# peterhpark/neuroclear

Measured on AMD Instinct MI355X. Metric: voxels/sec, higher is better.
Workload: dtype f32

## Files before the change

### include/nc_hip.h

```cpp
#ifndef NC_HIP_H
#define NC_HIP_H

#include <stddef.h>
#include <stdint.h>

#ifdef __cplusplus
extern "C" {
#endif

#define NC_OK 0
#define NC_ERR_SHAPE (-1)
#define NC_ERR_WS (-2)
#define NC_ERR_HIP (-3)
#define NC_ERR_ARG (-4)

const char* nc_last_error(void);
int nc_version(void);
int nc_conv_fwd_path(int C, int K, int kd, int kh, int kw, int stride, int pad);
int nc_conv_wgrad_path(int C, int K, int kd, int kh, int kw, int stride, int pad);
void nc_prof_begin(double min_flop);
int nc_prof_end(int max, int* cls, double* flop, float* ms);
int nc_prof_end2(int max, int* cls, double* flop, float* ms, double* abytes);
void nc_set_force_direct(int on);
void nc_sconv_set_cfg(int cfg);
// ... 146 lines not shown
size_t nc_unet_deconv_param_floats(void);
size_t nc_unet_deconv_saved_floats(int N, int S0, int S1, int S2);
size_t nc_unet_deconv_train_ws_bytes(int N, int S0, int S1, int S2);
int nc_unet_deconv_train_fwd(const float* params, const float* x, float* y, float* saved, int N, int S0, int S1, int S2,
                             void* ws, size_t ws_bytes, void* stream, unsigned* kept);
int nc_unet_deconv_bwd(const float* params, const float* x, const float* y, const float* saved, const float* dy, float* dx,
                       float* dparams, int N, int S0, int S1, int S2, void* ws, size_t ws_bytes, void* stream, unsigned kept);
void nc_set_unet_lean(int on);
int nc_get_unet_lean(void);
void nc_set_unet_wprep(int on);
int nc_get_unet_wprep(void);
int nc_unet_wprep_layout(int N, int S0, int S1, int S2, int block, int form, size_t* pack_off, size_t* pack_bytes, size_t* cell_off,
                         size_t* bound_off);
int nc_s3x_pack_h2_debug(const float* w, int C, int K, int form, const unsigned* cell_a, const unsigned* cell_b, void* wp, unsigned* wcell,
                         void* stream);
int nc_convT_h2_bound_debug(const float* w, const float* bias, int C, int K, float in_bound, unsigned* cell, void* stream);
size_t nc_deep_linear_param_floats(void);
size_t nc_deep_linear_saved_floats(int N, int S0, int S1, int S2);
size_t nc_deep_linear_ws_bytes(int N, int S0, int S1, int S2);
int nc_deep_linear_fwd(const float* params, const float* x, float* y, float* saved , int N, int S0, int S1,
                       int S2, void* ws, size_t ws_bytes, void* stream, unsigned* kept );
void nc_set_dl_collapse(int on);
int nc_get_dl_collapse(void);
int nc_deep_linear_bwd(const float* params, const float* x, const float* saved, const float* dy, float* dx, float* dparams,
                       int N, int S0, int S1, int S2, void* ws, size_t ws_bytes, void* stream, unsigned kept);

int nc_conv_fwd_c8(const void* xh, const float* w, const float* bias, void* yh, int out_ctot, int out_c0, int N, int C, int D, int H,
                   int W, int K, int kd, int kh, int kw, int stride, int pad, int dtype, void* ws, size_t ws_bytes, void* stream);
int nc_conv_dgrad_c8(const void* dyh, const float* w, void* dxh, int N, int C, int D, int H, int W, int K, int kd, int kh, int kw,
                     int stride, int pad, int dtype, void* ws, size_t ws_bytes, void* stream);
size_t nc_conv_c1_c8_ws_bytes(int N, int D, int H, int W, int ks);
int nc_conv_c1_fwd_c8(const float* x, const float* w, const float* bias, void* yh, int out_ctot, int out_c0, int N, int D, int H, int W,
                      int ks, int dtype, void* ws, size_t ws_bytes, void* stream);
int nc_conv_c1_dgrad_c8(const void* dyh, const float* w, float* dx, int N, int D, int H, int W, int ks, void* ws, size_t ws_bytes,
                        void* stream);
size_t nc_conv_c1_wgrad_c8_ws_bytes(int N, int D, int H, int W, int ks);
int nc_conv_c1_wgrad_c8(const float* x, const void* dyh, float* dw, int N, int D, int H, int W, int ks, void* ws, size_t ws_bytes,
                        void* stream);
size_t nc_c8_instnorm_ws_bytes(int N, int C, long S);
int nc_c8_instnorm_stats(const void* xh, int N, int C, long S, float eps, float* mean, float* rstd, int dtype, void* ws,
                         size_t ws_bytes, void* stream);
int nc_c8_instnorm_act_fwd(const void* xh, const float* mean, const float* rstd, float slope, void* yh, int out_ctot, int out_c0,
                           int N, int C, long S, int dtype, void* stream);
int nc_c8_instnorm_act_bwd(const void* gh, int g_ctot, int g_c0, const void* xh, const float* mean, const float* rstd, float slope,
                           void* dxh, float* dbias , int N, int C, long S, int dtype, void* ws, size_t ws_bytes,
                           void* stream);
// ... 99 lines not shown
```

### neuroclear_amd/_lib.py

```python
import ctypes
import os
import re

_HERE = os.path.dirname(os.path.abspath(__file__))
LIB_PATH = os.environ.get('NC_HIP_LIB') or os.path.join(_HERE, 'csrc', 'libnc_hip.so')
HEADER_PATH = os.path.join(os.path.dirname(_HERE), 'include', 'nc_hip.h')

_lib = None


class NcError(RuntimeError):
    pass


def header_symbols():
    src = open(HEADER_PATH).read()
    src = re.sub(r'/\*.*?\*/', '', src, flags=re.S)
    return sorted(set(re.findall(r'\b(nc_[a-zA-Z0-9_]+)\s*\(', src)))


def lib():
    global _lib
    if _lib is None:
        if not os.path.exists(LIB_PATH):
            raise NcError('libnc_hip.so is not built (%s): run `python -c "import __graft_entry__ as g; g.build()"` '
                          'or `make -C neuroclear_amd/csrc`; there is no CPU fallback' % LIB_PATH)
        L = ctypes.CDLL(LIB_PATH)
        for name in header_symbols():
            fn = getattr(L, name)
            if name.endswith('_bytes') or name.endswith('_floats') or name == 'nc_h2_cells_offset':
                fn.restype = ctypes.c_size_t
            elif name == 'nc_last_error':
                fn.restype = ctypes.c_char_p
            elif name in ('nc_set_force_direct', 'nc_prof_begin', 'nc_sconv_set_cfg', 'nc_sconv_set_tune', 'nc_set_conv_split', 'nc_set_s3_fusion', 'nc_set_c8x_mode', 'nc_set_split_terms', 'nc_set_h2_guard', 'nc_set_epi_stats', 'nc_set_dl_collapse', 'nc_set_p2d_terms', 'nc_set_s3x_w64', 'nc_set_unet_lean', 'nc_set_unet_wprep'):
                fn.restype = None
            else:
                fn.restype = ctypes.c_int
        _lib = L
    return _lib


def check(code, what=''):
    if code != 0:
        raise NcError('%s failed (%d): %s' % (what, code, lib().nc_last_error().decode()))


P = ctypes.c_void_p
I = ctypes.c_int
L_ = ctypes.c_long
F = ctypes.c_float
Z = ctypes.c_size_t
```

### neuroclear_amd/csrc/common.hpp

```cpp
#pragma once
#include <hip/hip_runtime.h>

#include <cstdarg>
#include <cstdio>

#include "../../include/nc_hip.h"

namespace nc {

void set_error(const char* fmt, ...);

inline int check_launch(const char* what) {
  hipError_t e = hipGetLastError();
  if (e != hipSuccess) {
    set_error("%s: %s", what, hipGetErrorString(e));
    return NC_ERR_HIP;
  }
  return NC_OK;
}

inline long cdiv(long a, long b) { return (a + b - 1) / b; }

int raise_dyn_lds(const void* kernel, int bytes, const char* who);
template <typename K>
// ... 174 lines not shown
struct WPrepSeg { const float* w; int Cin, Kout, flip; unsigned a_bits; int b_cell; unsigned* ext_cell; };
struct WPrepBound { const float* w; const float* bias; int C, K; float in_bound; int cell; };
size_t wprep_bytes(const WPrepSeg* segs, int n);
int wprep_run(const WPrepSeg* segs, int n, const WPrepBound* bounds, int nb, void* region, S3xPrepared* out, hipStream_t s);
int s3x_pack_h2(const float* w, int Cin, int Kout, int KS, long so, long si, int flip, int split_c, const unsigned* cell_a, const unsigned* cell_b,
                unsigned* wcell, void* wp_ws, hipStream_t s);
void s3x_set_terms(int t);
int s3x_get_terms();
int conv_s3x_h2(const void* xs, const unsigned* cell_a, const unsigned* cell_b, int split_c, const float* w, const float* bias, float* y, int N,
                int Cin, int D, int H, int W, int Kout, int KS, long so, long si, int flip, unsigned* wcell, void* wp_ws, hipStream_t s,
                const unsigned* guard = nullptr, float* stats_part = nullptr, const S3xPrepared* prep = nullptr);
size_t s3x_stats_bytes(int N, int D, int H, int W, int Kout, int KS);
int s3x_stats_finalize(const float* stats_part, const float* bias, int N, int D, int H, int W, int Kout, int KS, float eps, float* mean, float* rstd,
                       hipStream_t s);
bool c1k7_h2_supported(const ConvDims& d);
size_t c1k7_h2_ws_bytes(const ConvDims& d);
int conv_c1k7_h2(const float* x, const float* w, const float* bias, float* y, const ConvDims& d, void* ws, size_t wsb, hipStream_t s);
size_t c1k7_h2_dgrad_ws_bytes(const ConvDims& d);
bool dl_typed_supported(int N, int D, int H, int W);
size_t dl_typed_bytes(int N, int D, int H, int W);
const float* dl_typed_wp(const char* scratch, int N, int D, int H, int W);
float* dl_typed_dwsw(char* scratch, int N, int D, int H, int W);
int dl_typed_compose(const float* F, char* scratch, int N, int D, int H, int W, hipStream_t s);
int dl_typed_fwd_boundary(const float* act0, float* y, char* scratch, int N, int D, int H, int W, hipStream_t s);
int dl_typed_dgrad_boundary(const float* act0, const float* dy, float* g, char* scratch, int N, int D, int H, int W, hipStream_t s);
int dl_typed_p(const float* act0, const float* dy, float* Pq, char* scratch, int N, int D, int H, int W, hipStream_t s);
int conv_c1k7_h2_dgrad(const float* dy, const float* w, float* dx, const ConvDims& d, void* ws, size_t wsb, hipStream_t s);
inline size_t h2_cells_offset(size_t elems) { return (elems * 4 + 255) & ~(size_t)255; }
inline unsigned* h2_cells_of(const void* t, size_t elems) { return (unsigned*)((char*)const_cast<void*>(t) + h2_cells_offset(elems)); }
int instnorm_relu_tail_sigmoid(const float* x, const float* mean, const float* rstd, const float* w1, const float* b1, const float* w2,
                               const float* b2, float* y, int C, long S, hipStream_t s);
int instnorm_act_bwd_dbias_h2(const float* dy, const float* x, const float* mean, const float* rstd, float slope, void* dxs,
                              float* dbias, int N, int C, long S, void* ws, size_t ws_bytes, void* stream, unsigned* guard = nullptr);
int instnorm_act_bwd_dbias_h2_rank1(const float* dy1, const float* w1, const float* x, const float* mean, const float* rstd, float slope, void* dxs,
                                    float* dbias, int C, long S, void* ws, size_t ws_bytes, void* stream, unsigned* guard);
unsigned* conv_bwd_guard_words(void* ws, int N, int K, long S);
int maxpool2_h2(const void* in, void* out, int N, int C, int ctot, int D, int H, int W, hipStream_t s);
int h2_zero_cells(unsigned* cells, int n, hipStream_t s);
int h2_set_cell(unsigned* cell, float bound, hipStream_t s);
int h2_absmax(const float* x, long n, unsigned* cell, hipStream_t s, unsigned* cell2 = nullptr);
int split2h_into(const float* x, long xstride, void* xs, int N, int C, long S, int ctot, int c0, const unsigned* cell, hipStream_t s,
                 unsigned* guard = nullptr);
constexpr int kGuardLow = 0, kGuardAll = 1, kGuardFlag = 2;
constexpr unsigned kGuardDrop = 17u << 23;
constexpr unsigned long long kGuardShare = 64;
#if defined(__HIP_DEVICE_COMPILE__)
__device__ __forceinline__ bool guard_skip(const unsigned* guard, int want) {
  return guard && (int)(__builtin_nontemporal_load(guard + kGuardFlag) != 0) != want;
}
// ... 113 lines not shown
```

### neuroclear_amd/csrc/dl_typed.hip

```cpp
#include "common.hpp"

namespace nc {
namespace {

constexpr int kT = 27, kD7 = 343, kC = 64;

__host__ __device__ inline int axis_type(int coord, int L) { return coord == 0 ? 0 : coord == L - 1 ? 2 : 1; }
__host__ __device__ inline bool tap_ok(int ta, int t) { return !((ta == 0 && t == 0) || (ta == 2 && t == 2)); }

__global__ void __launch_bounds__(64) k_dl_h_from_f(const float* __restrict__ F, float* __restrict__ Hc, float* __restrict__ Hd, float* __restrict__ Wp,
                                                    float* __restrict__ Hr, float* __restrict__ Hx) {
  const int tau = blockIdx.x, d = blockIdx.y, c = threadIdx.x;
  const int dz = d / 49, dy = (d / 7) % 7, dx = d % 7;
  const int tz_ = tau / 9, ty_ = (tau / 3) % 3, tx_ = tau % 3;
  double v = 0.0, v13 = 0.0;
  for (int tz = 0; tz < 3; ++tz) {
    const int sz = dz - tz;
    if (sz < 0 || sz > 4) continue;
    for (int ty = 0; ty < 3; ++ty) {
      const int sy = dy - ty;
      if (sy < 0 || sy > 4) continue;
      for (int tx = 0; tx < 3; ++tx) {
        const int sx = dx - tx;
        if (sx < 0 || sx > 4) continue;
// ... 347 lines not shown
  const int tau = blockIdx.y;
  const long i = (long)blockIdx.x * 256 + threadIdx.x;
  if (i >= (long)kD7 * kC) return;
  const int tz = tau / 9, ty = (tau / 3) % 3, tx = tau % 3;
  double v = 0.0;
  if (tau != 13) {
    for (int n = 0; n < N; ++n) {
      if (tx == 1) {
        int r0, cnt, st;
        if (tz != 1) { const int b = tz == 0 ? 0 : H; r0 = b + (ty == 0 ? 0 : ty == 2 ? H - 1 : 1); cnt = ty == 1 ? H - 2 : 1; st = 1; }
        else { r0 = 2 * H + (ty == 2 ? 1 : 0); cnt = D - 2; st = 2; }
        for (int j = 0; j < cnt; ++j) v += (double)partA[((long)n * nrows + r0 + (long)j * st) * kD7 * kC + i];
      } else {
        const int side = tx >> 1;
        const long slot = (long)N * 2 * D * kD7 * kC;
        const int z0 = tz == 0 ? 0 : tz == 2 ? D - 1 : 1, cnt = tz == 1 ? D - 2 : 1;
        for (int j = 0; j < cnt; ++j) v += (double)partB[(long)ty * slot + (((long)n * 2 + side) * D + z0 + j) * kD7 * kC + i];
      }
    }
  }
  dHb[(long)tau * kD7 * kC + i] = (float)v;
}

size_t al256(size_t b) { return (b + 255) & ~(size_t)255; }

}

struct DlTyped {
  size_t Hc, Hd, Wp, dWsw, dHb, AX, dyX, partA, partB, Hr, Hx, total;
  int nrows;
};
static DlTyped dl_typed_plan(int N, int D, int H, int W) {
  DlTyped t{};
  size_t off = 0;
  auto take = [&](size_t b) { const size_t r = off; off += al256(b); return r; };
  t.nrows = n_bnd_rows(D, H);
  t.Hc = take((size_t)kT * kD7 * kC * 4); t.Hd = take((size_t)kT * kD7 * kC * 4); t.Wp = take((size_t)kC * kD7 * 4); t.dWsw = take((size_t)kC * kD7 * 4);
  t.dHb = take((size_t)kT * kD7 * kC * 4);
  t.AX = take((size_t)N * 2 * kC * D * 4 * H * 4); t.dyX = take((size_t)N * 2 * D * H * 4);
  t.Hr = take((size_t)kT * 49 * kC * 8 * 4); t.Hx = take((size_t)kT * 49 * kC * 8 * 4);
  t.partA = take((size_t)N * t.nrows * kD7 * kC * 4); t.partB = take((size_t)3 * N * 2 * D * kD7 * kC * 4);
  t.total = off;
  return t;
}
bool dl_typed_supported(int N, int D, int H, int W) {
  return N >= 1 && D >= 8 && H >= 8 && W >= 8 && H <= 192 && W <= 192 && W % 4 == 0;
}
size_t dl_typed_bytes(int N, int D, int H, int W) { return dl_typed_supported(N, D, H, W) ? dl_typed_plan(N, D, H, W).total : 0; }
const float* dl_typed_wp(const char* scratch, int N, int D, int H, int W) { return (const float*)(scratch + dl_typed_plan(N, D, H, W).Wp); }
float* dl_typed_dwsw(char* scratch, int N, int D, int H, int W) { return (float*)(scratch + dl_typed_plan(N, D, H, W).dWsw); }

int dl_typed_compose(const float* F, char* scratch, int N, int D, int H, int W, hipStream_t s) {
  const DlTyped t = dl_typed_plan(N, D, H, W);
  hipLaunchKernelGGL(k_dl_h_from_f, dim3(kT, kD7), dim3(64), 0, s, F, (float*)(scratch + t.Hc), (float*)(scratch + t.Hd), (float*)(scratch + t.Wp), (float*)(scratch + t.Hr),
                     (float*)(scratch + t.Hx));
  return check_launch("deep_linear: typed kernels");
}
int dl_typed_fwd_boundary(const float* act0, float* y, char* scratch, int N, int D, int H, int W, hipStream_t s) {
  const DlTyped t = dl_typed_plan(N, D, H, W);
  float* AX = (float*)(scratch + t.AX);
  hipLaunchKernelGGL(k_dl_gather_x, dim3((unsigned)D, kC, (unsigned)(N * 2)), dim3(128), 0, s, act0, AX, (const float*)nullptr, (float*)nullptr, D, H, W);
  hipLaunchKernelGGL(k_dl_bnd_fwd<false>, dim3((unsigned)t.nrows, (unsigned)cdiv(W - 2, kSeg), (unsigned)N), dim3(448), 0, s, act0, (const float*)(scratch + t.Hr), y, D, H, W);
  hipLaunchKernelGGL(k_dl_bnd_fwd<true>, dim3((unsigned)D, (unsigned)(2 * cdiv(H - 2, kSeg)), (unsigned)N), dim3(448), 0, s, (const float*)AX, (const float*)(scratch + t.Hx), y,
                     D, H, W);
  hipLaunchKernelGGL(k_dl_bnd_fwd_ends, dim3((unsigned)D, 4, (unsigned)N), dim3(256), 0, s, (const float*)AX, (const float*)(scratch + t.Hc), y, D, H, W);
  return check_launch("deep_linear: typed forward, boundary");
}
int dl_typed_dgrad_boundary(const float* act0, const float* dy, float* g, char* scratch, int N, int D, int H, int W, hipStream_t s) {
  const DlTyped t = dl_typed_plan(N, D, H, W);
  float* AX = (float*)(scratch + t.AX);
  float* dyX = (float*)(scratch + t.dyX);
  hipLaunchKernelGGL(k_dl_gather_x, dim3((unsigned)D, kC, (unsigned)(N * 2)), dim3(128), 0, s, act0, AX, dy, dyX, D, H, W);
  hipLaunchKernelGGL(k_dl_bnd_dgrad<false>, dim3((unsigned)(D * H), (unsigned)cdiv(W, 64), (unsigned)N), dim3(256), 0, s, dy, (const float*)(scratch + t.Hd), g, D, H, W, 1);
  const int nseg = (int)cdiv(H, 64);
  hipLaunchKernelGGL(k_dl_bnd_dgrad<true>, dim3((unsigned)D, 2, (unsigned)(N * nseg)), dim3(256), 0, s, (const float*)dyX, (const float*)(scratch + t.Hd), g, D, H, W, nseg);
  hipLaunchKernelGGL(k_dl_bnd_dgrad_ends, dim3((unsigned)D, 4, (unsigned)N), dim3(256), 0, s, (const float*)dyX, (const float*)(scratch + t.Hd), g, D, H, W);
  return check_launch("deep_linear: typed data gradient, boundary");
}
int dl_typed_p(const float* act0, const float* dy, float* Pq, char* scratch, int N, int D, int H, int W, hipStream_t s) {
  const DlTyped t = dl_typed_plan(N, D, H, W);
  const float* AX = (const float*)(scratch + t.AX);
  const float* dyX = (const float*)(scratch + t.dyX);
  const size_t lds = (size_t)(64 * kPitch + 192) * 4;
  hipLaunchKernelGGL(k_dl_bnd_wgrad<false>, dim3((unsigned)t.nrows, 7, (unsigned)N), dim3(448), lds, s, act0, dy, (float*)(scratch + t.partA), D, H, W, t.nrows);
  hipLaunchKernelGGL(k_dl_bnd_wgrad<true>, dim3((unsigned)(2 * D), 7, (unsigned)N), dim3(448), lds, s, AX, dyX, (float*)(scratch + t.partB), D, H, W, t.nrows);
  hipLaunchKernelGGL(k_dl_bnd_reduce, dim3((unsigned)cdiv((long)kD7 * kC, 256), kT), dim3(256), 0, s, (const float*)(scratch + t.partA), (const float*)(scratch + t.partB),
                     (float*)(scratch + t.dHb), N, D, H, W, t.nrows);
  hipLaunchKernelGGL(k_dl_p_from_dh, dim3(kC, 32), dim3(128), 0, s, (const float*)(scratch + t.dWsw), (const float*)(scratch + t.dHb), Pq);
  return check_launch("deep_linear: typed parameter gradients");
}

}
```

### neuroclear_amd/csrc/gen_nets.hip

```cpp

#include <atomic>
#include <cstdlib>

#include "common.hpp"

using namespace nc;

#define NC_TRY(expr) do { int e_ = (expr); if (e_) return e_; } while (0)

namespace {

size_t up64(size_t n) { return (n + 63) & ~(size_t)63; }

size_t s3_floats(size_t elems) { return up64((elems * 6 + 3) / 4); }
size_t align256(size_t b) { return (b + 255) & ~(size_t)255; }

std::atomic<int> g_unet_lean{getenv("NC_UNET_LEAN") ? (atoi(getenv("NC_UNET_LEAN")) != 0) : 1};
constexpr int kLeanBit0 = 10;
constexpr int kLeanBlocks[5] = {1, 3, 5, 6, 8};
int lean_index(int consumer) {
  for (int j = 0; j < 5; ++j) if (kLeanBlocks[j] == consumer) return j;
  return -1;
}

// ... 586 lines not shown
  const int t = threadIdx.x;
  const double* a = (const double*)(tail + LTail::a);
  const double* r = (const double*)(tail + LTail::r);
  for (int i = t; i < 32 * 64; i += 256) dw3[i] = (float)(a[i / 64] * r[i % 64]);
  if (t < 32) {
    double v = 0.0;
    for (int c = 0; c < 64; ++c) v += (double)w3[t * 64 + c] * r[c];
    ss[t] = v;
  }
  __syncthreads();
  for (int i = t; i < 16 * 32; i += 256) dw4[i] = (float)((double)w5[i / 32] * ss[i % 32]);
  if (t < 16) {
    double v = 0.0;
    for (int b = 0; b < 32; ++b) v += (double)w4[t * 32 + b] * ss[b];
    dw5[t] = (float)v;
  }
}

std::atomic<int> g_dl_collapse{getenv("NC_DL_COLLAPSE") ? (atoi(getenv("NC_DL_COLLAPSE")) < 0 ? 0 : atoi(getenv("NC_DL_COLLAPSE")) > 2 ? 2 : atoi(getenv("NC_DL_COLLAPSE"))) : 2};

}

namespace nc {
bool dl_collapse_on() { return g_dl_collapse.load(std::memory_order_relaxed) != 0; }
size_t dl_tail_bytes() { return LTail::bytes; }
const float* dl_tail_E(const char* tail) { return (const float*)(tail + LTail::E); }
const float* dl_tail_Ef(const char* tail) { return (const float*)(tail + LTail::Ef); }
float* dl_tail_q(char* tail) { return (float*)(tail + LTail::q); }
int dl_tail_compose(const float* w2, const float* w3, const float* w4, const float* w5, char* tail, hipStream_t s) {
  hipLaunchKernelGGL(k_dl_compose, dim3(8), dim3(256), 0, s, w2, w3, w4, w5, tail);
  return check_launch("deep_linear: compose");
}
float* dl_tail_P(char* tail) { return (float*)(tail + LTail::P); }
const float* dl_w1_fold(char* tail, const float* w1, hipStream_t s) {
  hipLaunchKernelGGL(k_dl_w1_fold, dim3(64, 32), dim3(128), 0, s, (const float*)(tail + LTail::E), w1, (float*)(tail + LTail::Wf));
  return check_launch("deep_linear_bwd: composed data-gradient weights") ? nullptr : (const float*)(tail + LTail::Wf);
}
const float* dl_fold_fwd64(char* tail, const float* w1, hipStream_t s) {
  static_assert(LTail::Wf == LTail::P + (size_t)64 * 32 * 125 * 4 + 256, "P and Wf adjacent");
  float* F = (float*)(tail + LTail::P);
  if (hipMemsetAsync(F + (size_t)32 * 64 * 125, 0, (size_t)32 * 64 * 125 * 4, s) != hipSuccess) return nullptr;
  hipLaunchKernelGGL(k_dl_fold_fwd, dim3(32, 64), dim3(128), 0, s, (const float*)(tail + LTail::E), w1, F);
  return check_launch("deep_linear_fwd: composed forward weights") ? nullptr : F;
}
int dl_combine27(const float* Z, float* y, int N, int D, int H, int W, int zch, hipStream_t s) {
  hipLaunchKernelGGL(k_dl_combine27, dim3(1024, (unsigned)N), dim3(256), 0, s, Z, y, D, H, W, zch);
// ... 44 lines not shown
  return true;
}

}

extern "C" {

size_t nc_deep_linear_param_floats(void) {
  LPlan p;
  l_plan(p, 1, 8, 8, 8);
  return p.params;
}

size_t nc_deep_linear_saved_floats(int N, int S0, int S1, int S2) {
  LPlan p;
  return l_plan(p, N, S0, S1, S2) ? p.saved : 0;
}

size_t nc_deep_linear_ws_bytes(int N, int S0, int S1, int S2) {
  LPlan p;
  return l_plan(p, N, S0, S1, S2) ? align256(p.conv_ws) + p.grads * sizeof(float) + 256 + align256(LTail::bytes) + dl_typed_bytes(N, S0, S1, S2) : 0;
}

void nc_set_dl_collapse(int on) { g_dl_collapse.store(on < 0 ? 0 : on > 2 ? 2 : on, std::memory_order_relaxed); }
int nc_get_dl_collapse(void) { return g_dl_collapse.load(std::memory_order_relaxed); }

int nc_deep_linear_fwd(const float* params, const float* x, float* y, float* saved, int N, int S0, int S1, int S2, void* ws,
                       size_t ws_bytes, void* stream, unsigned* kept) {
  NetworkScope net_scope;
  if (!params || !x || !y) { set_error("deep_linear_fwd: null pointer"); return NC_ERR_ARG; }
  LPlan p;
  if (!l_plan(p, N, S0, S1, S2)) { set_error("deep_linear_fwd: bad shape"); return NC_ERR_SHAPE; }
  if (!ws || ws_bytes < nc_deep_linear_ws_bytes(N, S0, S1, S2)) { set_error("deep_linear_fwd: workspace too small"); return NC_ERR_WS; }
  void* cws = ws;
  float* G = (float*)((char*)ws + align256(p.conv_ws));
  const float* in = x;
  unsigned kept_mask = 0;
  if (kept) *kept = 0;
  const bool collapse = g_dl_collapse.load(std::memory_order_relaxed) != 0;
  char* tail = (char*)ws + align256(p.conv_ws) + p.grads * sizeof(float) + 256;
  hipStream_t hs = (hipStream_t)stream;
  static const bool k32_on = !(getenv("NC_DL_K32") && atoi(getenv("NC_DL_K32")) == 0);
  char* typed = tail + align256(LTail::bytes);
  ConvDims d0;
  const bool typed_ok = g_dl_collapse.load(std::memory_order_relaxed) == 2 && saved && dl_typed_supported(N, S0, S1, S2) && make_dims(d0, N, 1, S0, S1, S2, 64, 7, 7, 7, 1, 3) && c1k7_h2_supported(d0) &&
                        c1_wgrad_supported(d0) && c1k7_h2_dgrad_ws_bytes(d0) <= p.conv_ws && c1k7_h2_ws_bytes(d0) <= p.conv_ws &&
                        c1_wgrad_ws_bytes(d0) <= p.conv_ws;
  for (int i = 0; i < 6; ++i) {
    ConvDims dk;
    if (typed_ok && i == 1) {
      hipLaunchKernelGGL(k_dl_compose, dim3(8), dim3(256), 0, hs, params + p.w[2], params + p.w[3], params + p.w[4], params + p.w[5], tail);
      hipLaunchKernelGGL(k_dl_fold_fwd, dim3(32, 64), dim3(128), 0, hs, (const float*)(tail + LTail::E), params + p.w[1], (float*)(tail + LTail::Wf));
      NC_TRY(check_launch("deep_linear_fwd: composed kernels"));
      NC_TRY(dl_typed_compose((const float*)(tail + LTail::Wf), typed, N, S0, S1, S2, hs));
      NC_TRY(conv_c1k7_h2_dgrad(in, dl_typed_wp(typed, N, S0, S1, S2), y, d0, cws, p.conv_ws, hs));
      NC_TRY(dl_typed_fwd_boundary(in, y, typed, N, S0, S1, S2, hs));
      kept_mask |= kKeptCollapsed | kKeptNoAct1 | kKeptTyped;
      break;
    }
    if (collapse && i == 1 && saved && k32_on && make_dims(dk, N, 64, S0, S1, S2, 32, 5, 5, 5, 1, 2) && conv_fwd_h2_k32_supported(dk) &&
        (size_t)256 + s3x_packed_bytes(64, 32, 5, 2) + 512 <= p.conv_ws) {
      hipLaunchKernelGGL(k_dl_compose, dim3(8), dim3(256), 0, hs, params + p.w[2], params + p.w[3], params + p.w[4], params + p.w[5], tail);
      hipLaunchKernelGGL(k_dl_fold_fwd, dim3(32, 64), dim3(128), 0, hs, (const float*)(tail + LTail::E), params + p.w[1], (float*)(tail + LTail::Wf));
      NC_TRY(check_launch("deep_linear_fwd: composed forward weights"));
      float* Z = saved + p.act[1];
      NC_TRY(conv_fwd_h2_k32_keep(in, (const float*)(tail + LTail::Wf), Z, dk, cws, p.conv_ws, hs, saved + p.xs3[1]));
      hipLaunchKernelGGL(k_dl_combine27, dim3(1024, (unsigned)N), dim3(256), 0, hs, (const float*)Z, y, S0, S1, S2, 32);
      NC_TRY(check_launch("deep_linear_fwd: shifted sum"));
      kept_mask |= kKeptCollapsed | kKeptNoAct1 | (1u << 1) | (1u << 17);
      break;
    }
    if (collapse && i == 2) {
      hipLaunchKernelGGL(k_dl_compose, dim3(8), dim3(256), 0, hs, params + p.w[2], params + p.w[3], params + p.w[4], params + p.w[5], tail);
      NC_TRY(check_launch("deep_linear_fwd: compose"));
      NC_TRY(conv_fwd_to1_k3(in, (const float*)(tail + LTail::E), y, N, 64, S0, S1, S2, cws, p.conv_ws, hs));
      kept_mask |= kKeptCollapsed;
      break;
    }
    const LLayer& l = kLL[i];
// ... 18 lines not shown
  NetworkScope net_scope;
  if (!params || !x || !saved || !dy || !dparams) { set_error("deep_linear_bwd: null pointer"); return NC_ERR_ARG; }
  LPlan p;
  if (!l_plan(p, N, S0, S1, S2)) { set_error("deep_linear_bwd: bad shape"); return NC_ERR_SHAPE; }
  if (!ws || ws_bytes < nc_deep_linear_ws_bytes(N, S0, S1, S2)) { set_error("deep_linear_bwd: workspace too small"); return NC_ERR_WS; }
  void* cws = ws;
  float* G = (float*)((char*)ws + align256(p.conv_ws));
  const float* g = dy;
  const unsigned kept_mask = kept;
  int top = 5;
  ConvDims dsh, cd1;
  static const bool rank_on = !(getenv("NC_DL_RANK_WGRAD") && atoi(getenv("NC_DL_RANK_WGRAD")) == 0);
  static const bool rank_dg_on = !(getenv("NC_DL_RANK_DGRAD") && atoi(getenv("NC_DL_RANK_DGRAD")) == 0);
  const bool h2_1 = make_dims(cd1, N, 64, S0, S1, S2, 64, 5, 5, 5, 1, 2) && conv_layer_h2(cd1);
  const bool have1 = ((kept_mask >> 1) & 1) && ((kept_mask >> 17) & 1) != 0;
  const bool rank_w = (kept_mask & kKeptCollapsed) && rank_on && h2_1 && have1 && make_dims(dsh, N, 32, S0, S1, S2, 64, 5, 5, 5, 1, 2) &&
                      wgrad_h2_supported(dsh) && s3_wgrad_ws_bytes(dsh) <= p.conv_ws;
  const bool rank_dgrad = rank_w && rank_dg_on && conv_fwd_h2_c32_supported(dsh) && conv_fwd_h2_c32_ws_bytes(dsh) <= p.conv_ws;
  const bool rank_all = rank_dgrad;
  if (kept_mask & kKeptTyped) {
    hipStream_t hs = (hipStream_t)stream;
    char* tail = (char*)ws + align256(p.conv_ws) + p.grads * sizeof(float) + 256;
    char* typed = tail + align256(LTail::bytes);
    ConvDims d0;
    ForceTwoTerm two_;
    if (!dl_typed_supported(N, S0, S1, S2) || !make_dims(d0, N, 1, S0, S1, S2, 64, 7, 7, 7, 1, 3) || !c1k7_h2_supported(d0) || !c1_wgrad_supported(d0)) {
      set_error("deep_linear_bwd: the forward ran the position-typed form, which this shape does not admit");
      return NC_ERR_ARG;
    }
    const float* act0 = saved + p.act[0];
    hipLaunchKernelGGL(k_dl_compose, dim3(8), dim3(256), 0, hs, params + p.w[2], params + p.w[3], params + p.w[4], params + p.w[5], tail);
    hipLaunchKernelGGL(k_dl_fold_fwd, dim3(32, 64), dim3(128), 0, hs, (const float*)(tail + LTail::E), params + p.w[1], (float*)(tail + LTail::Wf));
    NC_TRY(check_launch("deep_linear_bwd: composed kernels"));
    NC_TRY(dl_typed_compose((const float*)(tail + LTail::Wf), typed, N, S0, S1, S2, hs));
    float* g0 = G + p.g[1];
    NC_TRY(conv_c1k7_h2(dy, dl_typed_wp(typed, N, S0, S1, S2), nullptr, g0, d0, cws, p.conv_ws, hs));
    NC_TRY(dl_typed_dgrad_boundary(act0, dy, g0, typed, N, S0, S1, S2, hs));
    NC_TRY(conv_wgrad_c1(dy, act0, dl_typed_dwsw(typed, N, S0, S1, S2), d0, cws, p.conv_ws, hs));
    NC_TRY(dl_typed_p(act0, dy, (float*)(tail + LTail::P), typed, N, S0, S1, S2, hs));
    hipLaunchKernelGGL(k_dl_q_from_p, dim3(64, 27), dim3(256), 0, hs, params + p.w[1], (const float*)(tail + LTail::P), (float*)(tail + LTail::q));
    hipLaunchKernelGGL(k_dl_w1_contract, dim3(64, 64), dim3(128), 0, hs, (const float*)(tail + LTail::E), (const float*)(tail + LTail::P), dparams + p.w[1]);
    hipLaunchKernelGGL(k_dl_tail_w2, dim3(64), dim3(256), 0, hs, params + p.w[2], tail, dparams + p.w[2]);
    hipLaunchKernelGGL(k_dl_tail_w345, dim3(1), dim3(256), 0, hs, params + p.w[3], params + p.w[4], params + p.w[5], (const char*)tail, dparams + p.w[3],
                       dparams + p.w[4], dparams + p.w[5]);
    NC_TRY(check_launch("deep_linear_bwd: typed parameter gradients"));
    g = g0;
    top = 0;
  } else if (kept_mask & kKeptCollapsed) {
    hipStream_t hs = (hipStream_t)stream;
    char* tail = (char*)ws + align256(p.conv_ws) + p.grads * sizeof(float) + 256;
    const float* act1 = saved + p.act[1];
    hipLaunchKernelGGL(k_dl_compose, dim3(8), dim3(256), 0, hs, params + p.w[2], params + p.w[3], params + p.w[4], params + p.w[5], tail);
    NC_TRY(check_launch("deep_linear_bwd: compose"));
    if (rank_w) {
      float* Dsh = G + p.g[1];
      hipLaunchKernelGGL(k_dl_shift27, dim3(256, 32, (unsigned)N), dim3(256), 0, hs, dy, Dsh, S0, S1, S2);
      NC_TRY(check_launch("deep_linear_bwd: shifted copies of dy"));
      NC_TRY(conv_wgrad_h2(Dsh, nullptr, nullptr, saved + p.xs3[1], (float*)(tail + LTail::P), dsh, cws, p.conv_ws, hs));
      hipLaunchKernelGGL(k_dl_q_from_p, dim3(64, 27), dim3(256), 0, hs, params + p.w[1], (const float*)(tail + LTail::P), (float*)(tail + LTail::q));
      hipLaunchKernelGGL(k_dl_w1_contract, dim3(64, 64), dim3(128), 0, hs, (const float*)(tail + LTail::E), (const float*)(tail + LTail::P), dparams + p.w[1]);
      NC_TRY(check_launch("deep_linear_bwd: q, dW1"));
    } else {
// ... 50 lines not shown
```

Baseline: 55.04 million.

## Group boundary rows in typed deep-linear boundary kernels to reuse line loads

Adds grouped variants of the boundary forward, data-gradient and weight-gradient kernels for the position-typed deep-linear path. Each block now handles several adjacent boundary rows (kG=4) and reuses the loaded input lines and window shifts across them, instead of one row per block. The grouped path is on by default behind a new toggle. In exchange it uses more registers and LDS per block, adds decode logic, and runs fewer blocks.

```diff
diff --git a/include/nc_hip.h b/include/nc_hip.h
--- a/include/nc_hip.h
+++ b/include/nc_hip.h
@@ -192,6 +192,8 @@
                        int S2, void* ws, size_t ws_bytes, void* stream, unsigned* kept );
 void nc_set_dl_collapse(int on);
 int nc_get_dl_collapse(void);
+void nc_set_dl_bnd(int on);
+int nc_get_dl_bnd(void);
 int nc_deep_linear_bwd(const float* params, const float* x, const float* saved, const float* dy, float* dx, float* dparams,
                        int N, int S0, int S1, int S2, void* ws, size_t ws_bytes, void* stream, unsigned kept);
 
diff --git a/neuroclear_amd/_lib.py b/neuroclear_amd/_lib.py
--- a/neuroclear_amd/_lib.py
+++ b/neuroclear_amd/_lib.py
@@ -32,7 +32,7 @@
                 fn.restype = ctypes.c_size_t
             elif name == 'nc_last_error':
                 fn.restype = ctypes.c_char_p
-            elif name in ('nc_set_force_direct', 'nc_prof_begin', 'nc_sconv_set_cfg', 'nc_sconv_set_tune', 'nc_set_conv_split', 'nc_set_s3_fusion', 'nc_set_c8x_mode', 'nc_set_split_terms', 'nc_set_h2_guard', 'nc_set_epi_stats', 'nc_set_dl_collapse', 'nc_set_p2d_terms', 'nc_set_s3x_w64', 'nc_set_unet_lean', 'nc_set_unet_wprep'):
+            elif name in ('nc_set_force_direct', 'nc_prof_begin', 'nc_sconv_set_cfg', 'nc_sconv_set_tune', 'nc_set_conv_split', 'nc_set_s3_fusion', 'nc_set_c8x_mode', 'nc_set_split_terms', 'nc_set_h2_guard', 'nc_set_epi_stats', 'nc_set_dl_collapse', 'nc_set_p2d_terms', 'nc_set_s3x_w64', 'nc_set_unet_lean', 'nc_set_unet_wprep', 'nc_set_dl_bnd'):
                 fn.restype = None
             else:
                 fn.restype = ctypes.c_int
diff --git a/neuroclear_amd/csrc/common.hpp b/neuroclear_amd/csrc/common.hpp
--- a/neuroclear_amd/csrc/common.hpp
+++ b/neuroclear_amd/csrc/common.hpp
@@ -220,9 +220,9 @@
 const float* dl_typed_wp(const char* scratch, int N, int D, int H, int W);
 float* dl_typed_dwsw(char* scratch, int N, int D, int H, int W);
 int dl_typed_compose(const float* F, char* scratch, int N, int D, int H, int W, hipStream_t s);
-int dl_typed_fwd_boundary(const float* act0, float* y, char* scratch, int N, int D, int H, int W, hipStream_t s);
-int dl_typed_dgrad_boundary(const float* act0, const float* dy, float* g, char* scratch, int N, int D, int H, int W, hipStream_t s);
-int dl_typed_p(const float* act0, const float* dy, float* Pq, char* scratch, int N, int D, int H, int W, hipStream_t s);
+int dl_typed_fwd_boundary(const float* act0, float* y, char* scratch, int N, int D, int H, int W, bool groups, hipStream_t s);
+int dl_typed_dgrad_boundary(const float* act0, const float* dy, float* g, char* scratch, int N, int D, int H, int W, bool groups, hipStream_t s);
+int dl_typed_p(const float* act0, const float* dy, float* Pq, char* scratch, int N, int D, int H, int W, bool groups, hipStream_t s);
 int conv_c1k7_h2_dgrad(const float* dy, const float* w, float* dx, const ConvDims& d, void* ws, size_t wsb, hipStream_t s);
 inline size_t h2_cells_offset(size_t elems) { return (elems * 4 + 255) & ~(size_t)255; }
 inline unsigned* h2_cells_of(const void* t, size_t elems) { return (unsigned*)((char*)const_cast<void*>(t) + h2_cells_offset(elems)); }
diff --git a/neuroclear_amd/csrc/dl_typed.hip b/neuroclear_amd/csrc/dl_typed.hip
--- a/neuroclear_amd/csrc/dl_typed.hip
+++ b/neuroclear_amd/csrc/dl_typed.hip
@@ -393,6 +393,335 @@
   dHb[(long)tau * kD7 * kC + i] = (float)v;
 }
 
+constexpr int kG = 4;
+__device__ __forceinline__ int wave_id() { return __builtin_amdgcn_readfirstlane((int)(threadIdx.x >> 6)); }
+__host__ __device__ inline int n_groups(int L) { return (L - 2 + kG - 1) / kG; }
+__host__ __device__ inline int n_ygroups(int H) { return 2 * n_groups(H) + 4; }
+__host__ __device__ inline int n_zgroups(int D) { return 2 * n_groups(D); }
+__device__ inline void ygroup_decode(int g, int D, int H, int& vz, int& vy, int& cnt) {
+  const int ng = n_groups(H);
+  if (g < 2 * ng) { const int pl = g / ng; vz = pl ? D - 1 : 0; vy = 1 + (g - pl * ng) * kG; cnt = min(kG, H - 1 - vy); }
+  else { g -= 2 * ng; vz = (g & 2) ? D - 1 : 0; vy = (g & 1) ? H - 1 : 0; cnt = 1; }
+}
+__device__ inline void zgroup_decode(int g, int D, int H, int& vz, int& vy, int& cnt) {
+  const int ng = n_groups(D), e = g / ng;
+  vy = e ? H - 1 : 0; vz = 1 + (g - e * ng) * kG; cnt = min(kG, D - 1 - vz);
+}
+__device__ inline int row_index(int z, int y, int D, int H) { return z == 0 ? y : z == D - 1 ? H + y : 2 * H + 2 * (z - 1) + (y == H - 1 ? 1 : 0); }
+
+template <int MODE>
+__global__ void __launch_bounds__(MODE == 0 ? 448 : 64 * (kG + 6)) k_dl_bnd_fwd_g(const float* __restrict__ src, const float* __restrict__ Hl, float* __restrict__ y, int D,
+                                                                                 int H, int W) {
+  __shared__ float red[kG][7][64];
+  const int lane = threadIdx.x & 63, w = wave_id(), n = blockIdx.z;
+  const long HW = (long)H * W, S = (long)D * HW;
+  int vz, vy = 0, cnt, side = 0, seg, tau;
+  if constexpr (MODE == 0) { ygroup_decode(blockIdx.x, D, H, vz, vy, cnt); seg = blockIdx.y; tau = (axis_type(vz, D) * 3 + axis_type(vy, H)) * 3 + 1; }
+  else if constexpr (MODE == 1) { zgroup_decode(blockIdx.x, D, H, vz, vy, cnt); seg = blockIdx.y; tau = (3 + axis_type(vy, H)) * 3 + 1; }
+  else {
+    const int g = blockIdx.x, ng = n_groups(D);
+    if (g == 0) { vz = 0; cnt = 1; } else if (g == ng + 1) { vz = D - 1; cnt = 1; } else { vz = 1 + (g - 1) * kG; cnt = min(kG, D - 1 - vz); }
+    side = blockIdx.y & 1; seg = blockIdx.y >> 1; tau = axis_type(vz, D) * 9 + 3 + (side ? 2 : 0);
+  }
+  const int L = MODE == 2 ? H : W;
+  const int p = 1 + seg * kSeg + lane - 3;
+  const bool mine = lane >= 3 && lane < 3 + kSeg && p <= L - 2;
+  const bool inl = (unsigned)p < (unsigned)L;
+  const int zz = MODE == 0 ? vz + w - 3 : vz - 3 + w;
+  const long cs = MODE == 2 ? (long)D * 4 * H : S;
+  float a0[kG], a1[kG];
+#pragma unroll
+  for (int j = 0; j < kG; ++j) a0[j] = a1[j] = 0.f;
+  if ((unsigned)zz < (unsigned)D) {
+    const int nl = MODE == 0 ? cnt + 6 : MODE == 1 ? 7 : 4;
+    for (int t = 0; t < nl; ++t) {
+      const float* line;
+      if constexpr (MODE != 2) {
+        const int y2 = MODE == 0 ? vy - 3 + t : vy + t - 3;
+        if ((unsigned)y2 >= (unsigned)H) continue;
+        line = src + (long)n * kC * S + (long)zz * HW + (long)y2 * W;
+      } else {
+        line = src + ((long)n * 2 + side) * kC * cs + ((long)zz * 4 + t) * H;
+      }
+      const float4* h[kG];
+      bool ok[kG];
+#pragma unroll
+      for (int j = 0; j < kG; ++j) {
+        const int dzj = MODE == 0 ? w : w - j;
+        const int dq = MODE == 0 ? t - j : MODE == 1 ? t : (side ? t : t + 3);
+        ok[j] = j < cnt && (unsigned)dzj < 7u && (unsigned)dq < 7u;
+        h[j] = reinterpret_cast<const float4*>(Hl + (((long)tau * 7 + (ok[j] ? dzj : 0)) * 7 + (ok[j] ? dq : 0)) * kC * 8);
+      }
+      for (int c0 = 0; c0 < kC; c0 += 8) {
+        float v[8][7];
+#pragma unroll
+        for (int i = 0; i < 8; ++i) v[i][3] = inl ? line[(long)(c0 + i) * cs + p] : 0.f;
+#pragma unroll
+        for (int i = 0; i < 8; ++i) {
+          v[i][2] = dpp_prev(v[i][3]); v[i][1] = dpp_prev(v[i][2]); v[i][0] = dpp_prev(v[i][1]);
+          v[i][4] = dpp_next(v[i][3]); v[i][5] = dpp_next(v[i][4]); v[i][6] = dpp_next(v[i][5]);
+        }
+#pragma unroll
+        for (int j = 0; j < kG; ++j) {
+          if (!ok[j]) continue;
+#pragma unroll
+          for (int i = 0; i < 8; ++i) {
+            const float4 w0 = h[j][2 * (c0 + i)], w1 = h[j][2 * (c0 + i) + 1];
+            float& a = (i & 1) ? a1[j] : a0[j];
+            float& b = (i & 1) ? a0[j] : a1[j];
+            a = __builtin_fmaf(w0.x, v[i][0], a);
+            b = __builtin_fmaf(w0.y, v[i][1], b);
+            a = __builtin_fmaf(w0.z, v[i][2], a);
+            b = __builtin_fmaf(w0.w, v[i][3], b);
+            a = __builtin_fmaf(w1.x, v[i][4], a);
+            b = __builtin_fmaf(w1.y, v[i][5], b);
+            a = __builtin_fmaf(w1.z, v[i][6], a);
+          }
+        }
+      }
+    }
+  }
+#pragma unroll
+  for (int j = 0; j < kG; ++j) {
+    const int dzj = MODE == 0 ? w : w - j;
+    if ((unsigned)dzj < 7u) red[j][dzj][lane] = a0[j] + a1[j];
+  }
+  __syncthreads();
+  if (w < cnt && mine) {
+    float v = red[w][0][lane];
+#pragma unroll
+    for (int k = 1; k < 7; ++k) v += red[w][k][lane];
+    long o;
+    if constexpr (MODE == 0) o = (long)vz * HW + (long)(vy + w) * W + p;
+    else if constexpr (MODE == 1) o = (long)(vz + w) * HW + (long)vy * W + p;
+    else o = (long)(vz + w) * HW + (long)p * W + (side ? W - 1 : 0);
+    y[(long)n * S + o] = v;
+  }
+}
+
+template <bool XF>
+__global__ void __launch_bounds__(256) k_dl_bnd_dgrad_g(const float* __restrict__ dysrc, const float* __restrict__ Hd, float* __restrict__ g, int D, int H, int W,
+                                                        int nseg) {
+  const int lane = threadIdx.x & 63, q = wave_id();
+  const long HW = (long)H * W, S = (long)D * HW;
+  if constexpr (!XF) {
+    const int n = blockIdx.z;
+    int i = blockIdx.x, uz, uy;
+    if (i < 8 * H) { const int pz = i / H; uz = pz < 4 ? pz : D - 8 + pz; uy = i - pz * H; }
+    else { i -= 8 * H; const int e = i & 7; uz = 4 + (i >> 3); uy = e < 4 ? e : H - 8 + e; }
+    const int ux = blockIdx.y * kSeg + lane - 3;
+    const bool mine = lane >= 3 && lane < 3 + kSeg && ux < W;
+    const bool src_ok = ux >= 1 && ux <= W - 2;
+    float acc[16];
+#pragma unroll
+    for (int c = 0; c < 16; ++c) acc[c] = 0.f;
+    for (int dz = 0; dz < 7; ++dz) {
+      const int vz = uz - dz + 3;
+      if ((unsigned)vz >= (unsigned)D) continue;
+      const int tz = axis_type(vz, D);
+      for (int dy = 0; dy < 7; ++dy) {
+        const int vy = uy - dy + 3;
+        if ((unsigned)vy >= (unsigned)H) continue;
+        const int ty = axis_type(vy, H);
+        if (tz == 1 && ty == 1) continue;
+        const int tau = (tz * 3 + ty) * 3 + 1;
+        float s[7];
+        s[3] = src_ok ? dysrc[(long)n * S + (long)vz * HW + (long)vy * W + ux] : 0.f;
+        s[2] = dpp_next(s[3]); s[1] = dpp_next(s[2]); s[0] = dpp_next(s[1]);
+        s[4] = dpp_prev(s[3]); s[5] = dpp_prev(s[4]); s[6] = dpp_prev(s[5]);
+        const float* h0 = Hd + ((long)tau * kD7 + (dz * 7 + dy) * 7) * kC + q * 16;
+#pragma unroll
+        for (int dx = 0; dx < 7; ++dx) {
+          const float* h = h0 + dx * kC;
+#pragma unroll
+          for (int c = 0; c < 16; ++c) acc[c] = __builtin_fmaf(s[dx], h[c], acc[c]);
+        }
+      }
+    }
+    if (mine) {
+      float* o = g + ((long)n * kC + q * 16) * S + (long)uz * HW + (long)uy * W + ux;
+#pragma unroll
+      for (int c = 0; c < 16; ++c) o[(long)c * S] += acc[c];
+    }
+  } else {
+    const int uz = blockIdx.x, side = blockIdx.y;
+    const int n = blockIdx.z / nseg, seg = blockIdx.z - n * nseg;
+    const int uy = seg * 64 + lane;
+    const bool valid = uy < H;
+    const int tx = side ? 2 : 0;
+    float acc[4][16];
+#pragma unroll
+    for (int xr = 0; xr < 4; ++xr)
+#pragma unroll
+      for (int c = 0; c < 16; ++c) acc[xr][c] = 0.f;
+    for (int dz = 0; dz < 7; ++dz) {
+      const int vz = uz - dz + 3;
+      if ((unsigned)vz >= (unsigned)D) continue;
+      const int tau = (axis_type(vz, D) * 3 + 1) * 3 + tx;
+      const float* dpl = dysrc + (((long)n * 2 + side) * D + vz) * H;
+      for (int dy = 0; dy < 7; ++dy) {
+        const int vy = uy - dy + 3;
+        const bool in = valid && vy >= 1 && vy <= H - 2;
+        const float w = in ? dpl[vy] : 0.f;
+#pragma unroll
+        for (int xr = 0; xr < 4; ++xr) {
+          const int dx = side ? xr : xr + 3;
+          const float* h = Hd + ((long)tau * kD7 + (dz * 7 + dy) * 7 + dx) * kC + q * 16;
+#pragma unroll
+          for (int c = 0; c < 16; ++c) acc[xr][c] = __builtin_fmaf(w, h[c], acc[xr][c]);
+        }
+      }
+    }
+    if (valid) {
+      float4* o = reinterpret_cast<float4*>(g + ((long)n * kC + q * 16) * S + (long)uz * HW + (long)uy * W + (side ? W - 4 : 0));
+#pragma unroll
+      for (int c = 0; c < 16; ++c) {
+        float4 v = o[(long)c * (S / 4)];
+        v.x += acc[0][c]; v.y += acc[1][c]; v.z += acc[2][c]; v.w += acc[3][c];
+        o[(long)c * (S / 4)] = v;
+      }
+    }
+  }
+}
+
+__device__ __forceinline__ void dl_corr7(const float* __restrict__ a, const float* __restrict__ dyr, int L, float (&mid)[7]) {
+  float m0[7], m1[7];
+#pragma unroll
+  for (int k = 0; k < 7; ++k) m0[k] = m1[k] = 0.f;
+  auto guarded = [&](int x) __attribute__((always_inline)) {
+    const float d = dyr[x];
+#pragma unroll
+    for (int k = 0; k < 7; ++k) {
+      const int xs = x + k - 3, x0 = k < 2 ? 3 - k : 1;
+      if (xs < 0 || xs >= L) continue;
+      if ((x - x0) & 1) m1[k] = __builtin_fmaf(d, a[xs], m1[k]);
+      else m0[k] = __builtin_fmaf(d, a[xs], m0[k]);
+    }
+  };
+  int x = 1;
+  for (; x < 4; ++x) guarded(x);
+  float win[9];
+#pragma unroll
+  for (int k = 0; k < 7; ++k) win[k] = a[x - 3 + k];
+#pragma unroll 4
+  for (; x + 1 <= L - 5; x += 2) {
+    const float d0 = dyr[x], d1 = dyr[x + 1];
+    win[7] = a[x + 4]; win[8] = a[x + 5];
+#pragma unroll
+    for (int k = 0; k < 7; ++k) {
+      if (k == 1) { m0[k] = __builtin_fmaf(d0, win[k], m0[k]); m1[k] = __builtin_fmaf(d1, win[k + 1], m1[k]); }
+      else { m1[k] = __builtin_fmaf(d0, win[k], m1[k]); m0[k] = __builtin_fmaf(d1, win[k + 1], m0[k]); }
+    }
+#pragma unroll
+    for (int k = 0; k < 7; ++k) win[k] = win[k + 2];
+  }
+  for (; x <= L - 2; ++x) guarded(x);
+#pragma unroll
+  for (int k = 0; k < 7; ++k) mid[k] = m0[k] + m1[k];
+}
+template <bool XF>
+__global__ void __launch_bounds__(64 * kG) k_dl_bnd_wgrad_g(const float* __restrict__ asrc, const float* __restrict__ dysrc, float* __restrict__ part, int D, int H, int W,
+                                                           int nrows) {
+  extern __shared__ float lds[];
+  float* A = lds;
+  const int th = threadIdx.x, c = th & 63, j = wave_id();
+  float* dyr = lds + 64 * kPitch + j * 192;
+  const int f = blockIdx.y, n = blockIdx.z;
+  const long HW = (long)H * W, S = (long)D * HW;
+  const int L = XF ? H : W;
+  int vz, vy = 0, cnt, side = 0;
+  bool along_z = true;
+  if constexpr (!XF) {
+    const int g = blockIdx.x, ny = n_ygroups(H);
+    along_z = g >= ny;
+    if (!along_z) ygroup_decode(g, D, H, vz, vy, cnt); else zgroup_decode(g - ny, D, H, vz, vy, cnt);
+  } else {
+    side = blockIdx.x & 1; vz = (blockIdx.x >> 1) * kG; cnt = min(kG, D - vz);
+  }
+  const bool have = j < cnt;
+  const int rz = along_z ? vz + j : vz, ry = along_z ? vy : vy + j;
+  long pb = 0;
+  const long slot = XF ? (long)gridDim.z * 2 * D * kD7 * kC : 0;
+  if (have) {
+    const float* drow = XF ? dysrc + (((long)n * 2 + side) * D + rz) * H : dysrc + (long)n * S + (long)rz * HW + (long)ry * W;
+    for (int i = c; i < L; i += 64) dyr[i] = drow[i];
+    pb = XF ? (((long)n * 2 + side) * D + rz) * kD7 * kC + c : ((long)n * nrows + row_index(rz, ry, D, H)) * kD7 * kC + c;
+    if (XF && f == 0)
+      for (int dk = 0; dk < 49; ++dk)
+        for (int dxz = 0; dxz < 3; ++dxz) {
+          const long o = pb + (long)(dk * 7 + (side ? 4 + dxz : dxz)) * kC;
+          part[o] = 0.f; part[slot + o] = 0.f; part[2 * slot + o] = 0.f;
+        }
+  }
+  const long cs = XF ? (long)D * 4 * H : S;
+  constexpr int kCh = kC / kG, kXs = 3;
+  float st[kCh][kXs];
+  auto line_of = [&](int u, const float*& base) __attribute__((always_inline)) {
+    const int zz = XF ? vz - 3 + u : along_z ? vz - 3 + u : vz + f - 3;
+    const int y2 = XF ? 0 : along_z ? vy + f - 3 : vy - 3 + u;
+    if ((unsigned)zz >= (unsigned)D || (!XF && (unsigned)y2 >= (unsigned)H)) return false;
+    base = XF ? asrc + ((long)n * 2 + side) * kC * cs + ((long)zz * 4 + f) * H : asrc + (long)n * kC * S + (long)zz * HW + (long)y2 * W;
+    return true;
+  };
+  auto fetch = [&](int u) __attribute__((always_inline)) {
+    const float* base;
+    if (u >= cnt + 6 || !line_of(u, base)) return;
+#pragma unroll
+    for (int i = 0; i < kCh; ++i)
+#pragma unroll
+      for (int s = 0; s < kXs; ++s) {
+        const int xx = c + 64 * s;
+        st[i][s] = xx < L ? base[(long)(j + kG * i) * cs + xx] : 0.f;
+      }
+  };
+  fetch(0);
+  for (int u = 0; u < cnt + 6; ++u) {
+    const float* base;
+    const bool in = line_of(u, base);
+    if (in) {
+      __syncthreads();
+#pragma unroll
+      for (int i = 0; i < kCh; ++i)
+#pragma unroll
+        for (int s = 0; s < kXs; ++s) {
+          const int xx = c + 64 * s;
+          if (xx < L) A[(j + kG * i) * kPitch + xx] = st[i][s];
+        }
+      __syncthreads();
+    }
+    fetch(u + 1);
+    const int tw = u - j;
+    if (!have || (unsigned)tw >= 7u) continue;
+    float mid[7], e0[7], e1[7];
+#pragma unroll
+    for (int k = 0; k < 7; ++k) mid[k] = e0[k] = e1[k] = 0.f;
+    if (in) {
+      const float* a = A + c * kPitch;
+      dl_corr7(a, dyr, L, mid);
+      if constexpr (XF) {
+#pragma unroll
+        for (int k = 0; k < 7; ++k) {
+          const int sh = k - 3;
+          if (sh >= 0) e0[k] = dyr[0] * a[sh];
+          if (sh <= 0) e1[k] = dyr[H - 1] * a[H - 1 + sh];
+        }
+      }
+    }
+    if constexpr (!XF) {
+      const int dz = along_z ? tw : f, dy = along_z ? f : tw;
+#pragma unroll
+      for (int k = 0; k < 7; ++k) part[pb + (long)((dz * 7 + dy) * 7 + k) * kC] = mid[k];
+    } else {
+      const int dx = side ? f : f + 3;
+#pragma unroll
+      for (int k = 0; k < 7; ++k) {
+        const long o = pb + (long)((tw * 7 + k) * 7 + dx) * kC;
+        part[o] = e0[k]; part[slot + o] = mid[k]; part[2 * slot + o] = e1[k];
+      }
+    }
+  }
+}
+
 size_t al256(size_t b) { return (b + 255) & ~(size_t)255; }
 
 }
@@ -427,34 +756,59 @@
                      (float*)(scratch + t.Hx));
   return check_launch("deep_linear: typed kernels");
 }
-int dl_typed_fwd_boundary(const float* act0, float* y, char* scratch, int N, int D, int H, int W, hipStream_t s) {
+int dl_typed_fwd_boundary(const float* act0, float* y, char* scratch, int N, int D, int H, int W, bool groups, hipStream_t s) {
   const DlTyped t = dl_typed_plan(N, D, H, W);
   float* AX = (float*)(scratch + t.AX);
   hipLaunchKernelGGL(k_dl_gather_x, dim3((unsigned)D, kC, (unsigned)(N * 2)), dim3(128), 0, s, act0, AX, (const float*)nullptr, (float*)nullptr, D, H, W);
+  if (groups) {
+    const float* Hr = (const float*)(scratch + t.Hr);
+    hipLaunchKernelGGL(k_dl_bnd_fwd_g<0>, dim3((unsigned)n_ygroups(H), (unsigned)cdiv(W - 2, kSeg), (unsigned)N), dim3(448), 0, s, act0, Hr, y, D, H, W);
+    hipLaunchKernelGGL(k_dl_bnd_fwd_g<1>, dim3((unsigned)n_zgroups(D), (unsigned)cdiv(W - 2, kSeg), (unsigned)N), dim3(64 * (kG + 6)), 0, s, act0, Hr, y, D, H, W);
+    hipLaunchKernelGGL(k_dl_bnd_fwd_g<2>, dim3((unsigned)(n_groups(D) + 2), (unsigned)(2 * cdiv(H - 2, kSeg)), (unsigned)N), dim3(64 * (kG + 6)), 0, s, (const float*)AX,
+                       (const float*)(scratch + t.Hx), y, D, H, W);
+    hipLaunchKernelGGL(k_dl_bnd_fwd_ends, dim3((unsigned)D, 4, (unsigned)N), dim3(256), 0, s, (const float*)AX, (const float*)(scratch + t.Hc), y, D, H, W);
+    return check_launch("deep_linear: typed forward, boundary (row groups)");
+  }
   hipLaunchKernelGGL(k_dl_bnd_fwd<false>, dim3((unsigned)t.nrows, (unsigned)cdiv(W - 2, kSeg), (unsigned)N), dim3(448), 0, s, act0, (const float*)(scratch + t.Hr), y, D, H, W);
   hipLaunchKernelGGL(k_dl_bnd_fwd<true>, dim3((unsigned)D, (unsigned)(2 * cdiv(H - 2, kSeg)), (unsigned)N), dim3(448), 0, s, (const float*)AX, (const float*)(scratch + t.Hx), y,
                      D, H, W);
   hipLaunchKernelGGL(k_dl_bnd_fwd_ends, dim3((unsigned)D, 4, (unsigned)N), dim3(256), 0, s, (const float*)AX, (const float*)(scratch + t.Hc), y, D, H, W);
   return check_launch("deep_linear: typed forward, boundary");
 }
-int dl_typed_dgrad_boundary(const float* act0, const float* dy, float* g, char* scratch, int N, int D, int H, int W, hipStream_t s) {
+int dl_typed_dgrad_boundary(const float* act0, const float* dy, float* g, char* scratch, int N, int D, int H, int W, bool groups, hipStream_t s) {
   const DlTyped t = dl_typed_plan(N, D, H, W);
   float* AX = (float*)(scratch + t.AX);
   float* dyX = (float*)(scratch + t.dyX);
   hipLaunchKernelGGL(k_dl_gather_x, dim3((unsigned)D, kC, (unsigned)(N * 2)), dim3(128), 0, s, act0, AX, dy, dyX, D, H, W);
+  if (groups) {
+    const int nseg = (int)cdiv(H, 64);
+    hipLaunchKernelGGL(k_dl_bnd_dgrad_g<false>, dim3((unsigned)(8 * H + 8 * (D - 8)), (unsigned)cdiv(W, kSeg), (unsigned)N), dim3(256), 0, s, dy, (const float*)(scratch + t.Hd), g,
+                       D, H, W, 1);
+    hipLaunchKernelGGL(k_dl_bnd_dgrad_g<true>, dim3((unsigned)D, 2, (unsigned)(N * nseg)), dim3(256), 0, s, (const float*)dyX, (const float*)(scratch + t.Hd), g, D, H, W, nseg);
+    hipLaunchKernelGGL(k_dl_bnd_dgrad_ends, dim3((unsigned)D, 4, (unsigned)N), dim3(256), 0, s, (const float*)dyX, (const float*)(scratch + t.Hd), g, D, H, W);
+    return check_launch("deep_linear: typed data gradient, boundary (row groups)");
+  }
   hipLaunchKernelGGL(k_dl_bnd_dgrad<false>, dim3((unsigned)(D * H), (unsigned)cdiv(W, 64), (unsigned)N), dim3(256), 0, s, dy, (const float*)(scratch + t.Hd), g, D, H, W, 1);
   const int nseg = (int)cdiv(H, 64);
   hipLaunchKernelGGL(k_dl_bnd_dgrad<true>, dim3((unsigned)D, 2, (unsigned)(N * nseg)), dim3(256), 0, s, (const float*)dyX, (const float*)(scratch + t.Hd), g, D, H, W, nseg);
   hipLaunchKernelGGL(k_dl_bnd_dgrad_ends, dim3((unsigned)D, 4, (unsigned)N), dim3(256), 0, s, (const float*)dyX, (const float*)(scratch + t.Hd), g, D, H, W);
   return check_launch("deep_linear: typed data gradient, boundary");
 }
-int dl_typed_p(const float* act0, const float* dy, float* Pq, char* scratch, int N, int D, int H, int W, hipStream_t s) {
+int dl_typed_p(const float* act0, const float* dy, float* Pq, char* scratch, int N, int D, int H, int W, bool groups,
+               hipStream_t s) {
   const DlTyped t = dl_typed_plan(N, D, H, W);
   const float* AX = (const float*)(scratch + t.AX);
   const float* dyX = (const float*)(scratch + t.dyX);
   const size_t lds = (size_t)(64 * kPitch + 192) * 4;
-  hipLaunchKernelGGL(k_dl_bnd_wgrad<false>, dim3((unsigned)t.nrows, 7, (unsigned)N), dim3(448), lds, s, act0, dy, (float*)(scratch + t.partA), D, H, W, t.nrows);
-  hipLaunchKernelGGL(k_dl_bnd_wgrad<true>, dim3((unsigned)(2 * D), 7, (unsigned)N), dim3(448), lds, s, AX, dyX, (float*)(scratch + t.partB), D, H, W, t.nrows);
+  if (groups) {
+    const size_t ldsg = (size_t)(64 * kPitch + kG * 192) * 4;
+    hipLaunchKernelGGL(k_dl_bnd_wgrad_g<false>, dim3((unsigned)(n_ygroups(H) + n_zgroups(D)), 7, (unsigned)N), dim3(64 * kG), ldsg, s, act0, dy, (float*)(scratch + t.partA), D,
+                       H, W, t.nrows);
+    hipLaunchKernelGGL(k_dl_bnd_wgrad_g<true>, dim3((unsigned)(2 * cdiv(D, kG)), 4, (unsigned)N), dim3(64 * kG), ldsg, s, AX, dyX, (float*)(scratch + t.partB), D, H, W, t.nrows);
+  } else {
+    hipLaunchKernelGGL(k_dl_bnd_wgrad<false>, dim3((unsigned)t.nrows, 7, (unsigned)N), dim3(448), lds, s, act0, dy, (float*)(scratch + t.partA), D, H, W, t.nrows);
+    hipLaunchKernelGGL(k_dl_bnd_wgrad<true>, dim3((unsigned)(2 * D), 7, (unsigned)N), dim3(448), lds, s, AX, dyX, (float*)(scratch + t.partB), D, H, W, t.nrows);
+  }
   hipLaunchKernelGGL(k_dl_bnd_reduce, dim3((unsigned)cdiv((long)kD7 * kC, 256), kT), dim3(256), 0, s, (const float*)(scratch + t.partA), (const float*)(scratch + t.partB),
                      (float*)(scratch + t.dHb), N, D, H, W, t.nrows);
   hipLaunchKernelGGL(k_dl_p_from_dh, dim3(kC, 32), dim3(128), 0, s, (const float*)(scratch + t.dWsw), (const float*)(scratch + t.dHb), Pq);
diff --git a/neuroclear_amd/csrc/gen_nets.hip b/neuroclear_amd/csrc/gen_nets.hip
--- a/neuroclear_amd/csrc/gen_nets.hip
+++ b/neuroclear_amd/csrc/gen_nets.hip
@@ -632,6 +632,7 @@
 }
 
 namespace nc {
+static std::atomic<int> g_dl_bnd{1};
 bool dl_collapse_on() { return g_dl_collapse.load(std::memory_order_relaxed) != 0; }
 size_t dl_tail_bytes() { return LTail::bytes; }
 const float* dl_tail_E(const char* tail) { return (const float*)(tail + LTail::E); }
@@ -722,6 +723,8 @@
   return l_plan(p, N, S0, S1, S2) ? align256(p.conv_ws) + p.grads * sizeof(float) + 256 + align256(LTail::bytes) + dl_typed_bytes(N, S0, S1, S2) : 0;
 }
 
+void nc_set_dl_bnd(int on) { g_dl_bnd.store(on != 0, std::memory_order_relaxed); }
+int nc_get_dl_bnd(void) { return g_dl_bnd.load(std::memory_order_relaxed); }
 void nc_set_dl_collapse(int on) { g_dl_collapse.store(on < 0 ? 0 : on > 2 ? 2 : on, std::memory_order_relaxed); }
 int nc_get_dl_collapse(void) { return g_dl_collapse.load(std::memory_order_relaxed); }
 
@@ -738,6 +741,7 @@
   unsigned kept_mask = 0;
   if (kept) *kept = 0;
   const bool collapse = g_dl_collapse.load(std::memory_order_relaxed) != 0;
+  const bool bnd_groups = g_dl_bnd.load(std::memory_order_relaxed) != 0;
   char* tail = (char*)ws + align256(p.conv_ws) + p.grads * sizeof(float) + 256;
   hipStream_t hs = (hipStream_t)stream;
   static const bool k32_on = !(getenv("NC_DL_K32") && atoi(getenv("NC_DL_K32")) == 0);
@@ -754,7 +758,7 @@
       NC_TRY(check_launch("deep_linear_fwd: composed kernels"));
       NC_TRY(dl_typed_compose((const float*)(tail + LTail::Wf), typed, N, S0, S1, S2, hs));
       NC_TRY(conv_c1k7_h2_dgrad(in, dl_typed_wp(typed, N, S0, S1, S2), y, d0, cws, p.conv_ws, hs));
-      NC_TRY(dl_typed_fwd_boundary(in, y, typed, N, S0, S1, S2, hs));
+      NC_TRY(dl_typed_fwd_boundary(in, y, typed, N, S0, S1, S2, bnd_groups, hs));
       kept_mask |= kKeptCollapsed | kKeptNoAct1 | kKeptTyped;
       break;
     }
@@ -819,6 +823,7 @@
     hipStream_t hs = (hipStream_t)stream;
     char* tail = (char*)ws + align256(p.conv_ws) + p.grads * sizeof(float) + 256;
     char* typed = tail + align256(LTail::bytes);
+    const bool bnd_groups = g_dl_bnd.load(std::memory_order_relaxed) != 0;
     ConvDims d0;
     ForceTwoTerm two_;
     if (!dl_typed_supported(N, S0, S1, S2) || !make_dims(d0, N, 1, S0, S1, S2, 64, 7, 7, 7, 1, 3) || !c1k7_h2_supported(d0) || !c1_wgrad_supported(d0)) {
@@ -832,9 +837,9 @@
     NC_TRY(dl_typed_compose((const float*)(tail + LTail::Wf), typed, N, S0, S1, S2, hs));
     float* g0 = G + p.g[1];
     NC_TRY(conv_c1k7_h2(dy, dl_typed_wp(typed, N, S0, S1, S2), nullptr, g0, d0, cws, p.conv_ws, hs));
-    NC_TRY(dl_typed_dgrad_boundary(act0, dy, g0, typed, N, S0, S1, S2, hs));
+    NC_TRY(dl_typed_dgrad_boundary(act0, dy, g0, typed, N, S0, S1, S2, bnd_groups, hs));
     NC_TRY(conv_wgrad_c1(dy, act0, dl_typed_dwsw(typed, N, S0, S1, S2), d0, cws, p.conv_ws, hs));
-    NC_TRY(dl_typed_p(act0, dy, (float*)(tail + LTail::P), typed, N, S0, S1, S2, hs));
+    NC_TRY(dl_typed_p(act0, dy, (float*)(tail + LTail::P), typed, N, S0, S1, S2, bnd_groups, hs));
     hipLaunchKernelGGL(k_dl_q_from_p, dim3(64, 27), dim3(256), 0, hs, params + p.w[1], (const float*)(tail + LTail::P), (float*)(tail + LTail::q));
     hipLaunchKernelGGL(k_dl_w1_contract, dim3(64, 64), dim3(128), 0, hs, (const float*)(tail + LTail::E), (const float*)(tail + LTail::P), dparams + p.w[1]);
     hipLaunchKernelGGL(k_dl_tail_w2, dim3(64), dim3(256), 0, hs, params + p.w[2], tail, dparams + p.w[2]);
```

After: 55.32 million, median of 6. No clear change (+0.5%).
